# KleistLab/ADAPTed

Measured on AMD Instinct MI355X. Metric: reads/sec (adapter+polyA detect), RNA004 200k-sample reads, higher is better.
Workload: dtype f32 samples/statistics, f64 cumulative sums + LLR trace

## Files before the change

### adapted_amd/csrc/adapted_hip.hip

```cpp
#include <hip/hip_runtime.h>

#include <cmath>
#include <cstdio>
#include <cstring>
#include <cstdlib>
#include <string>
#include <vector>

#include "adapted_hip.h"
#include "handle.h"
#include "common.h"
__device__ unsigned long long g_dbg[ADP_NDBG] = {0};
__device__ unsigned long long g_bs_tally[ADP_NTALLY][8] = {{0}};
#include "llr_stream.h"
#include "n1_select.h"
#include "n1_fused.h"
#include "peaks.h"
#include "synth.h"
#include "validate.h"
#include "cand_stats2.h"
#include "series_pipe.h"
#include "cnn_topk.h"
#include "cnn_conv.h"
#include "cnn_conv_split.h"
// ... 64 lines not shown
    bad |= h->sp.ensure(R * sizeof(SpOut));
    bad |= h->any_none.ensure(64);
    h->vstride = ((h->m + 63) / 64) * 64;
    {
        size_t cap = (size_t)10000000000ull / ((size_t)8 * h->vstride);
        if (cap < 256) cap = 256;
        size_t want = R < 1024 * VAL_WPE ? R : 1024 * VAL_WPE;
        h->vslots = (int)(want < cap ? want : cap);
    }
    bad |= h->vscratch.ensure((size_t)h->vslots * 2 * h->vstride * 4);
    h->pslots = (int)(R < 8192 ? R : 8192);
    if (llr) {
    bad |= h->pk.ensure(R * (Lp / 2 + 1) * 4);
    if (env_int("ADP_PK_VALUES", 1)) bad |= h->pkv.ensure(R * (Lp / 2 + 1) * 8);
    bad |= h->npk.ensure(R * 4);
    bad |= h->mk.ensure((size_t)h->pslots * (Lp / 2 + 1) * 4);
    }
    ALLOCCHK(bad);
    return 0;
}

template <class SRC>
__global__ void __launch_bounds__(256) k_expand_ragged(const SRC *__restrict__ packed, const int64_t *__restrict__ offs,
                                                        const int32_t *__restrict__ full_len, const float *__restrict__ scale,
                                                        const float *__restrict__ offset, int m, float *__restrict__ out)
{
    const int r = blockIdx.y;
    const int i0 = (blockIdx.x * 256 + threadIdx.x) * 4;
    if (i0 >= m) return;
    const int len = full_len[r] < m ? (full_len[r] > 0 ? full_len[r] : 0) : m;
// ... 421 lines not shown
static inline SigIdx sig_subset(const SigF32 &s, const int32_t *sel) { return SigIdx{s.base, sel}; }
static inline SigIdxI16 sig_subset(const SigI16 &s, const int32_t *sel) { return SigIdxI16{s.base, s.scale, s.offset, s.full_len, sel}; }

static void launch_cumsum(adp_handle *h, int n)
{
    const int split = env_int("ADP_CUMSUM_GATHER", 1) != 0;
    hipLaunchKernelGGL(k_cumsum, dim3((n + 63) / 64), dim3(64), 0, h->stream, h->down.as<float>(), h->nvalid.as<int32_t>(), h->Lp, n,
                       h->nck, h->ck.as<double2>(), h->tail.as<double2>(), split);
    if (split)
        hipLaunchKernelGGL(k_cumsum_gather, dim3((n + 63) / 64), dim3(64), 0, h->stream, h->down.as<float>(), h->nvalid.as<int32_t>(), h->Lp, n,
                           h->nck, h->ck.as<double2>(), h->tail.as<double2>());
}

static int gains_tile_fast() { return env_int("ADP_GAINS_TILE_FAST", 1) != 0; }

static void launch_polya_peak(adp_handle *h, int n, int mbsize, const double *pkv)
{
    const int grid = n < h->pslots ? n : h->pslots;
    hipLaunchKernelGGL(k_polya_peak, dim3(grid), dim3(64), (size_t)(((h->Lp / 2 + 1) + 8) / 16 + 2) * 4, h->stream, h->trace.as<double>(), h->nvalid.as<int32_t>(), h->Lp,
                       h->bmax.as<double>(), h->bmin.as<double>(), h->nsum, h->adapter_idx.as<int32_t>(), n, mbsize, h->mbs.as<MbState>(),
                       h->pk.as<int32_t>(), h->mk.as<uint32_t>(), h->polya_idx.as<int32_t>(), h->npk.as<int32_t>(), pkv, env_int("ADP_PK_PREFIX", PK_PREFIX));
}

template <class SIG>
static int llr_enqueue(adp_handle *h, SIG dsig, const int32_t *dlen, int n, int m, int minibatch, int flags,
                       adp_row *rows_dev, int rows_kind , int32_t *mb_status_dev, double *mb_params_dev,
                       int upto, const PhaseSync *ps)
{
    int rc = 0;
    const int n_mb = (n + minibatch - 1) / minibatch;
    h->last_n = n; h->last_nmb = n_mb;
    ALLOCCHK(h->mbs.ensure((size_t)n_mb * sizeof(MbState)) || h->ghist.ensure((size_t)n_mb * N1_BINS * 4) || h->gbelow.ensure((size_t)n_mb * 8) || h->gcnt.ensure((size_t)n_mb * 8 * N1_NCNT));
    rc = alloc_all(h, n, true);
    if (rc) return rc;
    hipStream_t st = h->stream;
#ifdef ADP_ABLATE
// ... 66 lines not shown
        }
        if (upto >= 4) {
            Scope s(h, "k_gains<1>");
            hipLaunchKernelGGL(k_gains<1>, dim3((n + GAINS_WPB - 1) / GAINS_WPB), dim3(64 * GAINS_WPB), 0, st, h->down.as<float>(), h->nvalid.as<int32_t>(), h->Lp, h->nck,
                               h->ck.as<double2>(), h->tail.as<double2>(), h->adapter_idx.as<int32_t>(), minibatch, mbs,
                               h->trace.as<double>(), h->bmax.as<double>(), h->bmin.as<double>(), h->nsum, h->t1.as<int2>(), 0, h->pk.as<int32_t>(), h->npk.as<int32_t>(), h->Lp / 2 + 1, h->gstat.as<double>(), n, h->oh1, nullptr, gains_tile_fast());
        }
        if (upto >= 5) {
            Scope s(h, "k_adapter_peak");
            hipLaunchKernelGGL(k_adapter_peak, dim3(n), dim3(64), 0, st, h->trace.as<double>(), h->nvalid.as<int32_t>(), h->Lp,
                               h->bmax.as<double>(), h->bmin.as<double>(), h->nsum, h->t1.as<int2>(), minibatch, mbs,
                               h->cfg.adapter_peak_prominence, h->cfg.adapter_peak_rel_height,
                               h->cfg.adapter_peak_width / h->ds, h->adapter_idx.as<int32_t>(), h->gstat.as<double>());
        }
        double *pkvp = (env_int("ADP_PK_VALUES", 1) && h->pkv.cap >= (size_t)n * (h->Lp / 2 + 1) * 8) ? h->pkv.as<double>() : nullptr;
        if (upto >= 6) {
            Scope s(h, "k_gains<2>");
            hipLaunchKernelGGL(k_gains<2>, dim3((n + GAINS_WPB - 1) / GAINS_WPB), dim3(64 * GAINS_WPB), 0, st, h->down.as<float>(), h->nvalid.as<int32_t>(), h->Lp, h->nck,
                               h->ck.as<double2>(), h->tail.as<double2>(), h->adapter_idx.as<int32_t>(), minibatch, mbs,
                               h->trace.as<double>(), h->bmax.as<double>(), h->bmin.as<double>(), h->nsum, h->t1.as<int2>(), 0, h->pk.as<int32_t>(), h->npk.as<int32_t>(), h->Lp / 2 + 1, h->gstat.as<double>(), n, 5, pkvp, gains_tile_fast());
        }
        if (upto >= 7) {
            Scope s(h, "k_polya_peak");
            launch_polya_peak(h, n, minibatch, pkvp);
        }
        if (ps && ps->done[1]) HIPCHK(hipEventRecord(ps->done[1], st));
    }
    if (upto >= 8) {
        if (ps && ps->wait[2]) HIPCHK(hipStreamWaitEvent(st, ps->wait[2], 0));
        if (h->L > 0)
            hipLaunchKernelGGL(k_llr_bounds, dim3((n + 255) / 256), dim3(256), 0, st, h->adapter_idx.as<int32_t>(),
                               h->polya_idx.as<int32_t>(), n, h->ds, h->pos_off, h->bounds.as<int64_t>(), h->topk_none.as<int8_t>(), h->layout == ADP_LAYOUT_SINGLE_READ ? 1 : 0);
        rc = launch_validate(h, dsig, dlen, n, m, 1, minibatch, true);
        if (rc) return rc;
        if (flags & ADP_WITH_START_PEAK) {
            if (sp_forked) HIPCHK(hipStreamWaitEvent(st, h->ev_join, 0));
            else if (!sp_done) {
                Scope s(h, "k_start_peak");
                hipLaunchKernelGGL(k_start_peak<SIG>, dim3(n), dim3(64), (size_t)64 * h->cfg.sp_downscale_factor * 4, st, dsig, dlen, n, m, h->cfg, h->sp.as<SpOut>());
// ... 1415 lines not shown
        if (bytes < 12) return ADP_ERR_INVALID;
        int32_t c[3] = {0, 0, 0};
        if (h->pt_looked) { HIPCHK(hipMemcpyAsync(c, phase_counts(h, OPW_PT), 12, hipMemcpyDeviceToHost, h->stream)); HIPCHK(hipStreamSynchronize(h->stream)); }
        memcpy(host_out, c, 12); return ADP_OK; }
    case 9: src = h->have_series.p; if (bytes > h->have_series.cap) return ADP_ERR_INVALID; break;
    case 13: src = h->ck.p; if (bytes > h->ck.cap) return ADP_ERR_INVALID; break;
    case 14: src = h->tail.p; if (bytes > h->tail.cap) return ADP_ERR_INVALID; break;
    case 15: src = h->bmax.p; if (bytes > h->bmax.cap) return ADP_ERR_INVALID; break;
    case 16: src = h->bmin.p; if (bytes > h->bmin.cap) return ADP_ERR_INVALID; break;
    case 17: src = h->gstat.p; if (bytes > h->gstat.cap) return ADP_ERR_INVALID; break;
    case 18: src = h->npk.p; if (bytes > h->npk.cap) return ADP_ERR_INVALID; break;
    case 19: src = h->pk.p; if (bytes > h->pk.cap) return ADP_ERR_INVALID; break;
    case 20:
        if (!h->pkv.p) { g_err = "this handle keeps no heights beside its maxima lists (ADP_PK_VALUES=0)"; return ADP_ERR_INVALID; }
        src = h->pkv.p; if (bytes > h->pkv.cap) return ADP_ERR_INVALID; break;
    case 21: {
        if (h->last_grouped || !h->mbs.p || h->last_nmb < 1 || bytes > (uint64_t)h->last_nmb * 4 || h->gbelow.cap < (size_t)h->last_nmb * 4) return ADP_ERR_INVALID;
        hipLaunchKernelGGL(k_mb_status_out, dim3((h->last_nmb + 255) / 256), dim3(256), 0, h->stream, h->mbs.as<MbState>(), h->last_nmb, h->gbelow.as<int32_t>());
        src = h->gbelow.p; break; }
    case 8: { if (bytes < 64 || bytes > sizeof(unsigned long long) * ADP_NDBG) return ADP_ERR_INVALID;
              HIPCHK(hipMemcpyFromSymbol(host_out, HIP_SYMBOL(g_dbg), bytes, 0, hipMemcpyDeviceToHost));
              static unsigned long long tally[ADP_NTALLY][8];
              HIPCHK(hipMemcpyFromSymbol(tally, HIP_SYMBOL(g_bs_tally), sizeof(tally), 0, hipMemcpyDeviceToHost));
              unsigned long long *o = (unsigned long long *)host_out;
              for (int j = 0; j < 5; j++) { o[j] = 0; for (int i = 0; i < ADP_NTALLY; i++) o[j] += tally[i][j]; }
              return ADP_OK; }
    default: return ADP_ERR_INVALID;
    }
    if (!src || (what != 0 && h->last_grouped)) { g_err = "no stage buffers of a plain (one-group) LLR call on this handle"; return ADP_ERR_INVALID; }
    HIPCHK(hipMemcpyAsync(host_out, src, bytes, hipMemcpyDeviceToHost, h->stream));
// ... 7 lines not shown
```

### adapted_amd/csrc/find_peaks.h

```cpp
#pragma once
#include "common.h"

#define DBLMAX 1.7976931348623157e308

template <class P>
struct TraceViewT {
    P x;
    P bmax;
    P bmin;
    int lo, hi;
    int sanitize;
};
typedef TraceViewT<const double *> TraceView;
typedef TraceViewT<const LDS double *> TraceViewL;

template <class TV>
static __device__ __forceinline__ double tv_get(const TV &t, int i)
{
    double v = t.x[i];
    if (t.sanitize) {
        if (v != v) v = 0.0;
        else if (__builtin_isinf(v)) v = v > 0 ? DBLMAX : -DBLMAX;
    }
    return v;
// ... 88 lines not shown
        if (m) {
            found = bstart + __ffsll((long long)m) - 1;
            if (KIND == WALK_PROM && in && e < found && v < lmn) lmn = v;
            break;
        }
        if (KIND == WALK_PROM && in && v < lmn) lmn = v;
        i = bstart + SUMBLK;
    }
    if (KIND == WALK_PROM) mn = wave_min(lmn);
    return found;
}

#ifndef WALK_CHUNK
#define WALK_CHUNK 4
#endif
enum { PB_DONE = 0, PB_LEFT = 1, PB_RIGHT = 2, PB_REJECT = 4 };
template <class TV>
static __device__ int tv_prominence_budget(const TV &t, int p, int budget, double pmin, double &prom, double &lmin_out, double &rmin_out)
{
    const double xp = tv_get(t, p);
    double left_min = xp, right_min = xp;
    int more = 0;
    bool stopped = false;
    for (int i0 = p, steps = 0; !stopped && i0 >= t.lo; i0 -= WALK_CHUNK, steps += WALK_CHUNK) {
        if (steps >= budget) { more |= PB_LEFT; break; }
        double v[WALK_CHUNK];
#pragma unroll
        for (int u = 0; u < WALK_CHUNK; u++) v[u] = (i0 - u >= t.lo) ? tv_get(t, i0 - u) : 0.0;
#pragma unroll
        for (int u = 0; u < WALK_CHUNK; u++) {
            if (!stopped) {
                if (i0 - u < t.lo || !(v[u] <= xp)) stopped = true;
                else if (v[u] < left_min) left_min = v[u];
            }
        }
    }
    if (!(more & PB_LEFT) && !(pmin <= xp - left_min)) return PB_REJECT;
    stopped = false;
    for (int i0 = p, steps = 0; !stopped && i0 <= t.hi; i0 += WALK_CHUNK, steps += WALK_CHUNK) {
        if (steps >= budget) { more |= PB_RIGHT; break; }
        double v[WALK_CHUNK];
#pragma unroll
        for (int u = 0; u < WALK_CHUNK; u++) v[u] = (i0 + u <= t.hi) ? tv_get(t, i0 + u) : 0.0;
#pragma unroll
        for (int u = 0; u < WALK_CHUNK; u++) {
            if (!stopped) {
                if (i0 + u > t.hi || !(v[u] <= xp)) stopped = true;
                else if (v[u] < right_min) right_min = v[u];
            }
        }
    }
    if (!(more & PB_RIGHT) && !(pmin <= xp - right_min)) return PB_REJECT;
    prom = xp - (left_min > right_min ? left_min : right_min);
    lmin_out = left_min; rmin_out = right_min;
    return more;
}
template <class TV>
static __device__ bool tv_width_budget(const TV &t, int p, double prom, double rel, int budget, double &width, double lmin, double rmin)
{
    const double xp = tv_get(t, p);
    const double height = xp - prom * rel;
    int il = t.lo;
    {
        bool stopped = false;
        for (int i0 = p, steps = 0; !stopped && i0 > t.lo; i0 -= WALK_CHUNK, steps += WALK_CHUNK) {
            if (steps >= budget) return false;
            double v[WALK_CHUNK];
#pragma unroll
            for (int u = 0; u < WALK_CHUNK; u++) v[u] = (i0 - u > t.lo) ? tv_get(t, i0 - u) : 0.0;
#pragma unroll
            for (int u = 0; u < WALK_CHUNK; u++) {
                if (!stopped) {
                    if (i0 - u <= t.lo) { stopped = true; il = t.lo; }
                    else if (!(height < v[u]) || v[u] == lmin) { stopped = true; il = i0 - u; }
                }
            }
        }
    }
    int ir = t.hi;
    {
        bool stopped = false;
        for (int i0 = p, steps = 0; !stopped && i0 < t.hi; i0 += WALK_CHUNK, steps += WALK_CHUNK) {
            if (steps >= budget) return false;
            double v[WALK_CHUNK];
#pragma unroll
            for (int u = 0; u < WALK_CHUNK; u++) v[u] = (i0 + u < t.hi) ? tv_get(t, i0 + u) : 0.0;
#pragma unroll
            for (int u = 0; u < WALK_CHUNK; u++) {
                if (!stopped) {
                    if (i0 + u >= t.hi) { stopped = true; ir = t.hi; }
                    else if (!(height < v[u]) || v[u] == rmin) { stopped = true; ir = i0 + u; }
                }
            }
        }
    }
    double left_ip = (double)il, right_ip = (double)ir;
    { double xi = tv_get(t, il); if (xi < height) left_ip += (height - xi) / (tv_get(t, il + 1) - xi); }
    { double xi = tv_get(t, ir); if (xi < height) right_ip -= (height - xi) / (tv_get(t, ir - 1) - xi); }
    width = right_ip - left_ip;
    return true;
}

#ifndef WALK_BUDGET
#define WALK_BUDGET 8
#endif
template <class TV>
static __device__ bool wave_peak_ok(const TV &t, int p, double pmin, double wmin, double rel)
{
    const int ln = lane_id();
    double prom = 0.0, lmn = 0.0, rmn = 0.0;
    bool have = p >= 0, done = true;
    int pb = PB_DONE;
    if (have) pb = tv_prominence_budget(t, p, WALK_BUDGET, pmin, prom, lmn, rmn);
    if (pb == PB_REJECT) have = false;
// ... 23 lines not shown
        const double xp = tv_get(t, pp);
        const double height = xp - pr * rel;
        double dummy;
        int il = coop_find_down<WALK_WIDTH>(t, pp, t.lo + 1, xp, height, dummy, sl);
        if (il < t.lo + 1) il = t.lo;
        int ir = coop_find_up<WALK_WIDTH>(t, pp, t.hi - 1, xp, height, dummy, sr);
        if (ir > t.hi - 1) ir = t.hi;
        double left_ip = (double)il, right_ip = (double)ir;
        { double xi = tv_get(t, il); if (xi < height) left_ip += (height - xi) / (tv_get(t, il + 1) - xi); }
        { double xi = tv_get(t, ir); if (xi < height) right_ip -= (height - xi) / (tv_get(t, ir - 1) - xi); }
        if (ln == src) width = right_ip - left_ip;
    }
    return cand && (wmin <= width);
}

template <class TV>
static __device__ int wave_first_peak(const TV &t, double pmin, double wmin, double rel)
{
    const int ln = lane_id();
    for (int base = t.lo + 1; base < t.hi; base += 64) {
        int i = base + ln;
        int p = (i < t.hi) ? tv_peak_at(t, i) : -1;
        const bool ok = wave_peak_ok(t, p, pmin, wmin, rel);
        unsigned long long mk = __ballot(ok);
        if (mk) return __shfl(p, __ffsll((long long)mk) - 1);
    }
    return -1;
}
```

### adapted_amd/csrc/handle.h

```cpp
#pragma once
#include <hip/hip_runtime.h>

#include <string>
#include <vector>

#include "adapted_hip.h"
#include "carve.h"

#define ADP_HIDDEN __attribute__((visibility("hidden")))

extern ADP_HIDDEN thread_local std::string g_err;

#define HIPCHK(expr)                                                                         \
    do {                                                                                     \
        hipError_t e_ = (expr);                                                              \
        if (e_ != hipSuccess) {                                                              \
            g_err = std::string(#expr) + ": " + hipGetErrorString(e_);                       \
            return ADP_ERR_HIP;                                                              \
        }                                                                                    \
    } while (0)
#define RCCHK(expr) do { int rc_ = (expr); if (rc_) return rc_; } while (0)
#define ALLOCCHK(failed) do { if (failed) { g_err = "device allocation failed"; return ADP_ERR_HIP; } } while (0)

struct DevBuf {
// ... 18 lines not shown
struct ProfEntry { const char *name; hipEvent_t a, b; };
#define ADP_MAX_LANES 4

struct adp_handle {
    int device = 0;
    hipStream_t stream = nullptr;
    hipStream_t stream3 = nullptr;
    hipEvent_t ev_copy[16] = {};
    hipStream_t stream2 = nullptr;
    hipEvent_t ev_fork = nullptr, ev_join = nullptr;
    hipEvent_t ev_conv[3] = {};
    adp_cfg cfg;
    int max_reads = 0, m = 0;
    int T = 0, off = 0, ds = 1, L = 0, Lp = 0, nck = 0, nsum = 0;
    DevBuf mbs, ghist, gbelow, gcnt, cbuf, fz, fcnt, n1heavy, ct_pk, ct_pv, ct_out, gstat, down, nvalid, ck, tail, trace, bmax, bmin, t1, adapter_idx, polya_idx;
    DevBuf bounds, topk_none, rows, preq, series, have_series, vscratch, pk, pkv, npk, mk, st, sp, any_none, sig_stage, len_stage, bounds_stage;
    int vslots = 0, vstride = 0, pslots = 0;
    bool profiling = false;
    std::vector<ProfEntry> prof;
    std::vector<hipEvent_t> ev_pool;
    size_t ev_used = 0;
    int last_n = 0, last_nmb = 0;
    int layout = 0;
    int oh1 = 5;
    int pos_off = 0;
    DevBuf rng0;
    DevBuf cnn_w, cnn_act[2], cnn_x, cnn_sc, ct_st, ct_lnz, ct_ap, cstat, op_arena, op_used, series_plan;
    DevBuf ws;
    DevBuf fb_sel, so_sel, pt_sel, sub_ws;
    unsigned int fb_n_sel = 0, so_n_sel = 0;
    bool pt_looked = false;
// ... 57 lines not shown
```

### adapted_amd/csrc/llr_stream.h

```cpp
#pragma once
#include <type_traits>
#include "common.h"
#include "log_cr.h"
#include "wave_stats.h"

extern __device__ unsigned long long g_dbg[ADP_NDBG];

#define NP_TILE 512
struct SpHead {
    int32_t valid, max_idx, a2, e0;
    float mx;
    int32_t op_end;
    int32_t op_head, op_body, hit;
    int32_t pad;
};

template <class SIG, bool SP = false, int NQ = 0>
__global__ void __launch_bounds__(256) k_norm_pool(SIG sig, int m, int T, int off, int ds, int L, int Lp,
                                                   int mbsize, const MbState *__restrict__ mbs,
                                                   float *__restrict__ down, int32_t *__restrict__ nvalid,
                                                   const int64_t *__restrict__ ranges, const int32_t *__restrict__ full_len,
                                                   int tails_nan = 0, SpHead *__restrict__ sp_head = nullptr, float sp_thr = 0.f)
{
    extern __shared__ __attribute__((aligned(16))) float tile[];
// ... 323 lines not shown
#endif
#ifndef GAINS_EU
#define GAINS_EU 4
#endif
#ifndef GAINS_WPB
#define GAINS_WPB 4
#endif
template <int PASS>
__global__ void __launch_bounds__(64 * GAINS_WPB, 4) k_gains(const float *__restrict__ down, const int32_t *__restrict__ nvalid, int Lp, int nck,
                                              const double2 *__restrict__ ck, const double2 *__restrict__ tail,
                                              const int32_t *__restrict__ adapter_idx, int mbsize,
                                              const MbState *__restrict__ mbs, double *__restrict__ trace,
                                              double *__restrict__ bmax, double *__restrict__ bmin, int nsum,
                                              int2 *__restrict__ t1, int sanitize, int32_t *__restrict__ pk_all,
                                              int32_t *__restrict__ npk_all, int pk_stride, double *__restrict__ gstat, int n_reads, int oh1,
                                              double *__restrict__ pkv_all = nullptr, int tile_fast = 0)
{
    __shared__ __attribute__((aligned(16))) double sg_[GAINS_WPB][64 * (CK + 1)];
    __shared__ __attribute__((aligned(16))) double lt_[3 * LOGCR_N];
    LDS double *sg = (LDS double *)sg_[threadIdx.x >> 6];
    const int r = blockIdx.x * GAINS_WPB + (threadIdx.x >> 6);
    const int ln = lane_id();
    for (int i = threadIdx.x; i < 3 * LOGCR_N; i += 64 * GAINS_WPB) lt_[i] = g_logcr_table[i];
    __syncthreads();
    if (r >= n_reads) return;
    const LDS double *lt = (const LDS double *)lt_;
    auto flog = [&](double v) { return log_cr_impl(v, lt, [](double u) { return gains_log_slow(u); }); };
    if (mbs[r / mbsize].status != ADP_MB_OK) return;
    const int n = nvalid[r];
    if (n <= 0) return;
    int start = 0, oh = oh1, ot = 5;
    if (PASS == 2) {
        start = adapter_idx[r];
        if (start < 0) return;
        oh = 1; ot = 1;
    }
    const int E = n - 1;
    const float *s = down + (size_t)r * Lp;
    const double2 *c = ck + (size_t)r * nck;
// ... 11 lines not shown
    {
        double v = (start == E) ? 0.0 : var_seg(te.y, c2s, te.x, cs, (double)(E - start));
        vs = (double)(E - start) * flog(v);
    }
    const bool fast_read = tile_fast && __all(__builtin_fabs(vs) < __builtin_inf() && __builtin_bit_cast(uint64_t, vs) != 0x8000000000000000ULL);
    int n_fast = 0, n_redo = 0;
    int first_pos = 0x7fffffff, last_pos = -1;
    double st_s1 = 0.0, st_s2 = 0.0;
    int st_nan = 0;
    const bool emit = (PASS == 2 || sanitize) && pk_all;
    int32_t *pk = emit ? pk_all + (size_t)r * pk_stride : nullptr;
    double *pkv = (emit && pkv_all) ? pkv_all + (size_t)r * pk_stride : nullptr;
    int npk = 0;
    bool plateau = false;
    double carry1 = 0.0, carry2 = 0.0;
    for (int tb = 0; tb < n; tb += TRACE_TILE) {
        ws_sync();
        const int i0 = tb + ln * CK;
        const float4 *s4 = reinterpret_cast<const float4 *>(s + (i0 < Lp ? i0 : 0));
        double a = 0.0, b = 0.0;
        if (i0 < n) { double2 p = c[i0 / CK]; a = p.x; b = p.y; }
        double mx = -__builtin_inf(), mn = __builtin_inf();
        double dlh = (double)(i0 - start), dlt = (double)(E - i0);
        auto point = [&](auto interior_c, int t, int i, float qf) {
            constexpr bool INTERIOR = decltype(interior_c)::value;
            double gi = 0.0;
            const double lh_len = dlh, lt_len = dlt;
            dlh += 1.0; dlt -= 1.0;
            if (INTERIOR || i < n) {
                if (INTERIOR || (i >= start + oh && i < E - ot)) {
                    double vh = var_seg(b, c2s, a, cs, lh_len);
// ... 210 lines not shown
```

### adapted_amd/csrc/peaks.h

```cpp
#pragma once
#include "common.h"
#include "find_peaks.h"

extern __device__ unsigned long long g_dbg[ADP_NDBG];

template <class P>
static __device__ int adapter_peak_read(P g, P bmx, P bmn, int n, int2 se, double s1, double s2, int nnan,
                                        double prominence, double rel_height, int width)
{
    const int ln = lane_id();
    const int cn = se.y - se.x;
    if (n < 3 || cn < 3) return -1;
    double o1 = 0.0, o2 = 0.0; int onan = 0;
    for (int i0 = 0; i0 < se.x; i0 += 512) {
        double v[8];
#pragma unroll
        for (int u = 0; u < 8; u++) { const int i = i0 + u * 64 + ln; v[u] = i < se.x ? g[i] : 0.0; }
#pragma unroll
        for (int u = 0; u < 8; u++) { o1 += v[u]; o2 += v[u] * v[u]; }
    }
    for (int i0 = se.y; i0 < n; i0 += 512) {
        double v[8];
#pragma unroll
        for (int u = 0; u < 8; u++) { const int i = i0 + u * 64 + ln; v[u] = i < n ? g[i] : 0.0; }
// ... 58 lines not shown
#define PK_STEP 16
#endif
#ifndef PK_PREFIX
#define PK_PREFIX 224
#endif
#define PST_NONE 0u
#define PST_REMOVED 1u
#define PST_KEPT 2u
#define PST_UNDECIDED 3u

__global__ void __launch_bounds__(64, 8) k_polya_peak(const double *__restrict__ trace, const int32_t *__restrict__ nvalid, int Lp,
                                                   const double *__restrict__ bmax, const double *__restrict__ bmin, int nsum,
                                                   const int32_t *__restrict__ adapter_idx, int n_reads, int mbsize,
                                                   const MbState *__restrict__ mbs, int32_t *__restrict__ pk_all,
                                                   uint32_t *__restrict__ mk_all, int32_t *__restrict__ polya_idx,
                                                   const int32_t *__restrict__ npk_all, const double *__restrict__ pkv_all, int prefix)
{
    extern __shared__ __attribute__((aligned(16))) uint32_t stw_raw[];
    LDS uint32_t *stw = (LDS uint32_t *)stw_raw;
    const int ln = lane_id();
    const int half = Lp / 2 + 1;
    uint32_t *mk = mk_all + (size_t)blockIdx.x * half;
    for (int r = blockIdx.x; r < n_reads; r += gridDim.x) {
        int32_t *pk = pk_all + (size_t)r * half;
        int result = 0;
        const int n = nvalid[r];
        const bool active = mbs[r / mbsize].status == ADP_MB_OK && adapter_idx[r] >= 0 && n >= 3;
        if (active) {
            const double *g = trace + (size_t)r * Lp;
            TraceView tv{g, bmax + (size_t)r * nsum, bmin + (size_t)r * nsum, 0, n - 1, 1};
            int npk = npk_all[r];
            const bool recount = npk < 0;
            const double *pkv = (pkv_all && !recount) ? pkv_all + (size_t)r * half : nullptr;
            if (recount) npk = 0;
            double carry = 0.0;
            __syncthreads();
            for (int base0 = 0; recount && base0 < n; base0 += 256) {
                double vv[4], ee[4];
#pragma unroll
                for (int u = 0; u < 4; u++) {
                    const int i = base0 + u * 64 + ln;
                    vv[u] = (i < n) ? tv_get(tv, i) : 0.0;
                    ee[u] = (ln == 63 && i + 1 < n) ? tv_get(tv, i + 1) : 0.0;
                }
#pragma unroll
                for (int u = 0; u < 4; u++) {
                    const int base = base0 + u * 64;
                    if (base >= n) break;
                    const int i = base + ln;
                    const double v = vv[u];
                    double prev = __shfl_up(v, 1);
                    if (ln == 0) prev = carry;
                    double next = __shfl_down(v, 1);
                    if (ln == 63) next = ee[u];
                    carry = __shfl(v, 63);
                    int p = -1;
                    if (i > 0 && i < n - 1 && prev < v) {
                        if (next < v) p = i;
                        else if (next == v) {
                            int j = i + 1;
                            while (j < n - 1 && tv_get(tv, j) == v) j++;
                            if (tv_get(tv, j) < v) p = (i + j - 1) / 2;
                        }
                    }
                    unsigned long long m = __ballot(p >= 0);
                    if (p >= 0) pk[npk + __popcll(m & ((1ull << ln) - 1ull))] = p;
                    npk += __popcll(m);
                }
            }
            if (ABLATED(256)) npk = 0;
            int p0 = -1, p1 = -1;
            for (int attempt = 0; attempt < 2; attempt++) {
            const int wn = (attempt == 0 && prefix > 0 && npk > prefix) ? prefix : npk;
            __syncthreads();
            for (int w = ln; w < (wn + 8 + 15) / 16 + 1; w += 64) stw[w] = 0;
            __syncthreads();
            if (ln < 4 && wn + ln < npk) {
                const uint32_t sl = (uint32_t)(wn + ln + 4);
                __hip_atomic_fetch_or(&stw[sl >> 4], PST_UNDECIDED << ((sl & 15u) * 2u), __ATOMIC_RELAXED, __HIP_MEMORY_SCOPE_WORKGROUP);
            }
            int nund = 0;
            for (int base4 = 0; base4 < wn; base4 += 56 * 4) {
                int pp[4];
                double vv[4];
// ... 28 lines not shown
                    const double v = vv[u];
                    uint32_t mask = 0, lower = 0;
#pragma unroll
                    for (int j = 1; j <= 4; j++) {
                        const int pf = __shfl_down(p, j); const double vf = __shfl_down(v, j);
                        const bool within = pf - p <= 9;
                        if (within && vf >= v) mask |= 1u << (j - 1);
                        if (within && !(vf >= v)) lower |= 1u << (j - 1);
                    }
#pragma unroll
                    for (int j = 1; j <= 4; j++) {
                        const uint32_t lb = (uint32_t)__shfl_up((int)lower, j);
                        if (lb >> (j - 1) & 1u) mask |= 1u << (4 + j - 1);
                    }
                    const bool out = valid && ln >= 4 && ln < 60 && k < wn;
                    if (out) {
                        const uint32_t sl = (uint32_t)(k + 4);
                        __hip_atomic_fetch_or(&stw[sl >> 4], (mask ? PST_UNDECIDED : PST_KEPT) << ((sl & 15u) * 2u), __ATOMIC_RELAXED,
                                              __HIP_MEMORY_SCOPE_WORKGROUP);
                    }
                    const bool und = out && mask;
                    const unsigned long long m = __ballot(und);
                    if (und) mk[nund + __popcll(m & ((1ull << ln) - 1ull))] = ((uint32_t)k << 8) | mask;
                    nund += __popcll(m);
                }
            }
            __syncthreads();
            if (ABLATED(512)) nund = 0;
            while (nund > 0) {
                int w = 0;
                for (int base4 = 0; base4 < nund; base4 += 256) {
                    uint32_t ee[4];
#pragma unroll
                    for (int u = 0; u < 4; u++) { const int idx = base4 + 64 * u + ln; ee[u] = (idx < nund) ? mk[idx] : 0u; }
#pragma unroll
                    for (int u = 0; u < 4; u++) {
// ... 45 lines not shown
                    uint32_t stt = PST_NONE;
                    if (k < wn) {
                        const uint32_t sl = (uint32_t)(k + 4);
                        stt = (stw[sl >> 4] >> ((sl & 15u) * 2u)) & 3u;
                    }
                    const unsigned long long mu = __ballot(stt == PST_UNDECIDED);
                    if (mu && first_und == wn) first_und = base4 + 64 * u + __ffsll((long long)mu) - 1;
                    const bool kp = stt == PST_KEPT && k < first_und;
                    const unsigned long long m = __ballot(kp);
                    if (kp) kl[nkept + __popcll(m & ((1ull << ln) - 1ull))] = pq[u];
                    nkept += __popcll(m);
                }
            }
            __syncthreads();
            p0 = -1; p1 = -1;
            for (int base = 0; base < nkept && p1 < 0 && !ABLATED(1024); base += PK_STEP) {
                int k = base + ln;
                int i = (ln < PK_STEP && k < nkept) ? kl[k] : -1;
                const bool ok = wave_peak_ok(tv, i, 1.0, 10.0, 0.5);
                unsigned long long m = __ballot(ok);
                while (m && p1 < 0) {
                    int f = __ffsll((long long)m) - 1;
                    m &= m - 1;
                    int pi = __shfl(i, f);
                    if (p0 < 0) p0 = pi; else p1 = pi;
                }
            }
            if (p1 >= 0 || first_und >= npk) break;
            }
            if (p0 >= 0 && p1 < 0) result = p0;
            else if (p0 >= 0) {
                double h0 = g[p0], h1 = g[p1];
                if (h1 > h0) result = p1;
                else if (h1 < h0 * 0.5) result = p0;
                else {
                    double mv = __builtin_inf(); int mi = 0x7fffffff; int nan_i = 0x7fffffff;
                    for (int i = p0 + ln; i < p1; i += 64) {
                        double v = g[i];
                        if (v != v) nan_i = min(nan_i, i);
                        else if (v < mv) { mv = v; mi = i; }
                    }
                    nan_i = wave_min(nan_i);
                    double gm = wave_min(mv);
                    int cand = (mv == gm) ? mi : 0x7fffffff;
                    cand = wave_min(cand);
// ... 6 lines not shown
                    double xm = sx / cnt, ym = sy / cnt;
                    double sxx = 0, sxy = 0, syy = 0;
                    for (int i = idx_min + ln; i < p1; i += 64) {
                        double dx = (double)i - xm, dy = g[i] - ym;
                        sxx += dx * dx; sxy += dx * dy; syy += dy * dy;
                    }
                    sxx = wave_sum(sxx); sxy = wave_sum(sxy); syy = wave_sum(syy);
                    double inv = 1.0 / (double)cnt;
                    double ssxm = sxx * inv, ssxym = sxy * inv, ssym = syy * inv;
                    double rr;
                    if (ssxm == 0.0 || ssym == 0.0) rr = 0.0;
                    else { rr = ssxym / sqrt(ssxm * ssym); if (rr > 1.0) rr = 1.0; else if (rr < -1.0) rr = -1.0; }
                    result = (rr * rr >= 0.99) ? p1 : 0;
                }
            }
            __syncthreads();
        }
        if (ln == 0) polya_idx[r] = result;
    }
}
```

### adapted_amd/lib.py

```python
from __future__ import annotations

import ctypes as C
import operator
import os
import sys
from typing import List, Optional, Sequence

import numpy as np

from . import build as _build
from .container_types import DetectResults

_LIB = None

NCOL = 39
MAX_CAND = 16
MAX_OPEN_PORES = 16

ADP_IN_DEVICE, ADP_OUT_DEVICE, ADP_WITH_START_PEAK, ADP_TOPK_NONE, ADP_BOUNDS_HOST, ADP_TAILS_NAN = 1, 2, 4, 8, 16, 32
ADP_CNN_FALLBACK = 1 << 17
ADP_CNN_SECOND_LLR = 1 << 18
ADP_FLAG_TRUNCATED = 1 << 19
ADP_POLYA_TRUNCATED = 1 << 20
ROW_FROM_SECOND_LLR = 1
# ... 1235 lines not shown
    def debug_llr_upto(self, signals, full_lens, n, minibatch, stage, tails_nan: bool = False):
        sig, lens, flags = self._in(signals, full_lens, n, False)
        flags |= _flag_word(tails_nan=tails_nan)
        self._check(self.lib.adp_debug_llr_upto(self._h, sig, lens, n, self.m, int(minibatch), flags, int(stage)))

    def debug_fetch(self, what: int, n: int):
        lp = np.zeros(1, dtype=np.int32)
        self._check(self.lib.adp_debug_fetch(self._h, 6, lp, 4))
        Lp = int(lp[0])
        if what == 6:
            return Lp
        shapes = {1: ((n,), np.int32), 2: ((n, Lp), np.float32), 3: ((n, Lp), np.float64), 4: ((n,), np.int32),
                  5: ((n,), np.int32), 7: ((n, 2), np.int32), 9: ((n,), np.int8),
                  13: ((n, Lp // 16, 2), np.float64), 14: ((n, 2), np.float64), 15: ((n, Lp // 64), np.float64),
                  16: ((n, Lp // 64), np.float64), 17: ((n, 3), np.float64), 18: ((n,), np.int32),
                  19: ((n, Lp // 2 + 1), np.int32), 20: ((n, Lp // 2 + 1), np.float64), 21: ((n,), np.int32)}
        if what == 0:
            raise ValueError("use debug_norm_params")
        shp, dt = shapes[what]
        a = np.zeros(shp, dtype=dt)
        self._check(self.lib.adp_debug_fetch(self._h, what, a, a.nbytes))
        return a

    def debug_cnn_fallback(self):
        a = np.zeros(3, dtype=np.int32)
        self._check(self.lib.adp_debug_fetch(self._h, 10, a, a.nbytes))
        return tuple(int(v) for v in a)

    def debug_cnn_second_opinion(self):
        a = np.zeros(4, dtype=np.int32)
        self._check(self.lib.adp_debug_fetch(self._h, 11, a, a.nbytes))
# ... 17 lines not shown
```

Before: 1.077 million.

## Window the second gains pass and redo only reads with undecided polyA peaks

The second LLR gains pass now computes the trace only up to a fixed window past the adapter end. The polyA peak search runs on that truncated trace with window-aware prominence and width checks that can return an 'unknown' result. Reads whose answer cannot be decided inside the window go onto a redo list, and for those reads the full gains pass and peak search run again. This targets the cost of computing long traces past the likely polyA region, but it adds two extra kernel launches, a memset, atomics, and edge-case logic that could change results if the window checks are wrong.

```diff
diff --git a/adapted_amd/csrc/adapted_hip.hip b/adapted_amd/csrc/adapted_hip.hip
--- a/adapted_amd/csrc/adapted_hip.hip
+++ b/adapted_amd/csrc/adapted_hip.hip
@@ -102,6 +102,8 @@
     bad |= h->pk.ensure(R * (Lp / 2 + 1) * 4);
     if (env_int("ADP_PK_VALUES", 1)) bad |= h->pkv.ensure(R * (Lp / 2 + 1) * 8);
     bad |= h->npk.ensure(R * 4);
+    bad |= h->wend.ensure(R * 4);
+    bad |= h->redo.ensure((R + 1) * 4);
     bad |= h->mk.ensure((size_t)h->pslots * (Lp / 2 + 1) * 4);
     }
     ALLOCCHK(bad);
@@ -553,12 +555,29 @@
 
 static int gains_tile_fast() { return env_int("ADP_GAINS_TILE_FAST", 1) != 0; }
 
-static void launch_polya_peak(adp_handle *h, int n, int mbsize, const double *pkv)
+#define G2_WINDOW_DEFAULT 1024
+static int g2_window(int upto)
+{
+    const char *e = getenv("ADP_G2_WINDOW");
+    if (!e || !*e) return upto >= 8 ? G2_WINDOW_DEFAULT : 0;
+    const int w = env_int("ADP_G2_WINDOW", G2_WINDOW_DEFAULT);
+    return w < 0 ? 0 : (w > (1 << 28) ? (1 << 28) : w);
+}
+static void launch_gains2(adp_handle *h, int n, int mbsize, double *pkv, int win, const int32_t *redo)
+{
+    hipLaunchKernelGGL(k_gains<2>, dim3((n + GAINS_WPB - 1) / GAINS_WPB), dim3(64 * GAINS_WPB), 0, h->stream, h->down.as<float>(), h->nvalid.as<int32_t>(), h->Lp, h->nck,
+                       h->ck.as<double2>(), h->tail.as<double2>(), h->adapter_idx.as<int32_t>(), mbsize, h->mbs.as<MbState>(),
+                       h->trace.as<double>(), h->bmax.as<double>(), h->bmin.as<double>(), h->nsum, h->t1.as<int2>(), 0, h->pk.as<int32_t>(), h->npk.as<int32_t>(), h->Lp / 2 + 1, h->gstat.as<double>(), n, 5, pkv, gains_tile_fast(),
+                       win, h->wend.as<int32_t>(), redo);
+}
+
+static void launch_polya_peak(adp_handle *h, int n, int mbsize, const double *pkv, bool windowed = false, bool redo_pass = false)
 {
     const int grid = n < h->pslots ? n : h->pslots;
     hipLaunchKernelGGL(k_polya_peak, dim3(grid), dim3(64), (size_t)(((h->Lp / 2 + 1) + 8) / 16 + 2) * 4, h->stream, h->trace.as<double>(), h->nvalid.as<int32_t>(), h->Lp,
                        h->bmax.as<double>(), h->bmin.as<double>(), h->nsum, h->adapter_idx.as<int32_t>(), n, mbsize, h->mbs.as<MbState>(),
-                       h->pk.as<int32_t>(), h->mk.as<uint32_t>(), h->polya_idx.as<int32_t>(), h->npk.as<int32_t>(), pkv, env_int("ADP_PK_PREFIX", PK_PREFIX));
+                       h->pk.as<int32_t>(), h->mk.as<uint32_t>(), h->polya_idx.as<int32_t>(), h->npk.as<int32_t>(), pkv, env_int("ADP_PK_PREFIX", PK_PREFIX),
+                       (windowed || redo_pass) ? h->wend.as<int32_t>() : (const int32_t *)nullptr, (windowed || redo_pass) ? h->redo.as<int32_t>() : (int32_t *)nullptr, redo_pass ? 1 : 0);
 }
 
 template <class SIG>
@@ -655,15 +674,22 @@
                                h->cfg.adapter_peak_width / h->ds, h->adapter_idx.as<int32_t>(), h->gstat.as<double>());
         }
         double *pkvp = (env_int("ADP_PK_VALUES", 1) && h->pkv.cap >= (size_t)n * (h->Lp / 2 + 1) * 8) ? h->pkv.as<double>() : nullptr;
+        int win = g2_window(upto);
+        if (win > 0 && (win + 1 + TRACE_TILE - 1) / TRACE_TILE * TRACE_TILE >= h->L) win = 0;
         if (upto >= 6) {
+            if (win > 0) HIPCHK(hipMemsetAsync(h->redo.p, 0, 4, st));
             Scope s(h, "k_gains<2>");
-            hipLaunchKernelGGL(k_gains<2>, dim3((n + GAINS_WPB - 1) / GAINS_WPB), dim3(64 * GAINS_WPB), 0, st, h->down.as<float>(), h->nvalid.as<int32_t>(), h->Lp, h->nck,
-                               h->ck.as<double2>(), h->tail.as<double2>(), h->adapter_idx.as<int32_t>(), minibatch, mbs,
-                               h->trace.as<double>(), h->bmax.as<double>(), h->bmin.as<double>(), h->nsum, h->t1.as<int2>(), 0, h->pk.as<int32_t>(), h->npk.as<int32_t>(), h->Lp / 2 + 1, h->gstat.as<double>(), n, 5, pkvp, gains_tile_fast());
+            launch_gains2(h, n, minibatch, pkvp, win, nullptr);
         }
         if (upto >= 7) {
-            Scope s(h, "k_polya_peak");
-            launch_polya_peak(h, n, minibatch, pkvp);
+            { Scope s(h, "k_polya_peak");
+              launch_polya_peak(h, n, minibatch, pkvp, win > 0); }
+            if (win > 0) {
+                { Scope s(h, "k_gains<2> redo");
+                  launch_gains2(h, n, minibatch, pkvp, 0, h->redo.as<int32_t>()); }
+                { Scope s(h, "k_polya_peak redo");
+                  launch_polya_peak(h, n, minibatch, pkvp, false, true); }
+            }
         }
         if (ps && ps->done[1]) HIPCHK(hipEventRecord(ps->done[1], st));
     }
@@ -2109,6 +2135,8 @@
     case 20:
         if (!h->pkv.p) { g_err = "this handle keeps no heights beside its maxima lists (ADP_PK_VALUES=0)"; return ADP_ERR_INVALID; }
         src = h->pkv.p; if (bytes > h->pkv.cap) return ADP_ERR_INVALID; break;
+    case 22: src = h->wend.p; if (bytes > h->wend.cap) return ADP_ERR_INVALID; break;
+    case 23: src = h->redo.p; if (bytes > h->redo.cap) return ADP_ERR_INVALID; break;
     case 21: {
         if (h->last_grouped || !h->mbs.p || h->last_nmb < 1 || bytes > (uint64_t)h->last_nmb * 4 || h->gbelow.cap < (size_t)h->last_nmb * 4) return ADP_ERR_INVALID;
         hipLaunchKernelGGL(k_mb_status_out, dim3((h->last_nmb + 255) / 256), dim3(256), 0, h->stream, h->mbs.as<MbState>(), h->last_nmb, h->gbelow.as<int32_t>());
diff --git a/adapted_amd/csrc/find_peaks.h b/adapted_amd/csrc/find_peaks.h
--- a/adapted_amd/csrc/find_peaks.h
+++ b/adapted_amd/csrc/find_peaks.h
@@ -126,8 +126,8 @@
 #ifndef WALK_CHUNK
 #define WALK_CHUNK 4
 #endif
-enum { PB_DONE = 0, PB_LEFT = 1, PB_RIGHT = 2, PB_REJECT = 4 };
-template <class TV>
+enum { PB_DONE = 0, PB_LEFT = 1, PB_RIGHT = 2, PB_REJECT = 4, PB_OPEN = 8 };
+template <bool WIN = false, class TV>
 static __device__ int tv_prominence_budget(const TV &t, int p, int budget, double pmin, double &prom, double &lmin_out, double &rmin_out)
 {
     const double xp = tv_get(t, p);
@@ -149,6 +149,7 @@
     }
     if (!(more & PB_LEFT) && !(pmin <= xp - left_min)) return PB_REJECT;
     stopped = false;
+    bool higher = false;
     for (int i0 = p, steps = 0; !stopped && i0 <= t.hi; i0 += WALK_CHUNK, steps += WALK_CHUNK) {
         if (steps >= budget) { more |= PB_RIGHT; break; }
         double v[WALK_CHUNK];
@@ -157,17 +158,18 @@
 #pragma unroll
         for (int u = 0; u < WALK_CHUNK; u++) {
             if (!stopped) {
-                if (i0 + u > t.hi || !(v[u] <= xp)) stopped = true;
+                if (i0 + u > t.hi || !(v[u] <= xp)) { stopped = true; if (WIN && i0 + u <= t.hi) higher = true; }
                 else if (v[u] < right_min) right_min = v[u];
             }
         }
     }
-    if (!(more & PB_RIGHT) && !(pmin <= xp - right_min)) return PB_REJECT;
+    if (WIN && !(more & PB_RIGHT) && !higher) more |= PB_OPEN;
+    if (!(more & (WIN ? PB_RIGHT | PB_OPEN : PB_RIGHT)) && !(pmin <= xp - right_min)) return PB_REJECT;
     prom = xp - (left_min > right_min ? left_min : right_min);
     lmin_out = left_min; rmin_out = right_min;
     return more;
 }
-template <class TV>
+template <bool WIN = false, class TV>
 static __device__ bool tv_width_budget(const TV &t, int p, double prom, double rel, int budget, double &width, double lmin, double rmin)
 {
     const double xp = tv_get(t, p);
@@ -190,6 +192,7 @@
         }
     }
     int ir = t.hi;
+    bool crossed = false;
     {
         bool stopped = false;
         for (int i0 = p, steps = 0; !stopped && i0 < t.hi; i0 += WALK_CHUNK, steps += WALK_CHUNK) {
@@ -201,7 +204,7 @@
             for (int u = 0; u < WALK_CHUNK; u++) {
                 if (!stopped) {
                     if (i0 + u >= t.hi) { stopped = true; ir = t.hi; }
-                    else if (!(height < v[u]) || v[u] == rmin) { stopped = true; ir = i0 + u; }
+                    else if (!(height < v[u]) || v[u] == rmin) { stopped = true; ir = i0 + u; crossed = true; }
                 }
             }
         }
@@ -210,6 +213,7 @@
     { double xi = tv_get(t, il); if (xi < height) left_ip += (height - xi) / (tv_get(t, il + 1) - xi); }
     { double xi = tv_get(t, ir); if (xi < height) right_ip -= (height - xi) / (tv_get(t, ir - 1) - xi); }
     width = right_ip - left_ip;
+    if (WIN && !crossed) width = __builtin_nan("");
     return true;
 }
 
@@ -263,6 +267,93 @@
     return cand && (wmin <= width);
 }
 
+enum { PK3_FAIL = 0, PK3_PASS = 1, PK3_UNKNOWN = 2 };
+
+template <class TV>
+static __device__ double coop_width(const TV &t, int pp, double xp, double height, double sl, double sr, bool &crossed)
+{
+    double dummy;
+    int il = coop_find_down<WALK_WIDTH>(t, pp, t.lo + 1, xp, height, dummy, sl);
+    if (il < t.lo + 1) il = t.lo;
+    int ir = coop_find_up<WALK_WIDTH>(t, pp, t.hi - 1, xp, height, dummy, sr);
+    crossed = ir <= t.hi - 1;
+    if (!crossed) ir = t.hi;
+    double left_ip = (double)il, right_ip = (double)ir;
+    { double xi = tv_get(t, il); if (xi < height) left_ip += (height - xi) / (tv_get(t, il + 1) - xi); }
+    { double xi = tv_get(t, ir); if (xi < height) right_ip -= (height - xi) / (tv_get(t, ir - 1) - xi); }
+    return right_ip - left_ip;
+}
+
+template <class TV>
+static __device__ int wave_peak_ok_win(const TV &t, int p, double pmin, double wmin, double rel)
+{
+    const int ln = lane_id();
+    double prom = 0.0, lmn = 0.0, rmn = 0.0;
+    bool have = p >= 0;
+    int pb = PB_DONE;
+    if (have) pb = tv_prominence_budget<true>(t, p, WALK_BUDGET, pmin, prom, lmn, rmn);
+    if (pb == PB_REJECT) { have = false; pb = PB_DONE; }
+    unsigned long long todo = __ballot(have && (pb & (PB_LEFT | PB_RIGHT)));
+    while (todo) {
+        const int src = __ffsll((long long)todo) - 1;
+        todo &= todo - 1;
+        const int pp = __shfl(p, src), sides = __shfl(pb, src);
+        const double xp = tv_get(t, pp);
+        double lmin = __shfl(lmn, src), rmin = __shfl(rmn, src);
+        bool rej = false;
+        int open = sides & PB_OPEN;
+        if (sides & PB_LEFT) { coop_find_down<WALK_PROM>(t, pp, t.lo, xp, 0.0, lmin); rej = !(pmin <= xp - lmin); }
+        if (!rej && (sides & PB_RIGHT)) { if (coop_find_up<WALK_PROM>(t, pp, t.hi, xp, 0.0, rmin) > t.hi) open = PB_OPEN; }
+        if (ln == src) { if (rej) have = false; else { lmn = lmin; rmn = rmin; pb = open; } }
+    }
+    const double xpl = have ? tv_get(t, p) : 0.0;
+    const bool bounds = have && (pb & PB_OPEN) && rmn > lmn;
+    prom = xpl - (lmn > rmn ? lmn : rmn);
+    const bool cand = have && !bounds && (pmin <= prom);
+    int res = PK3_FAIL;
+    double width = 0.0;
+    bool done = true;
+    if (cand) done = tv_width_budget<true>(t, p, prom, rel, WALK_BUDGET, width, lmn, rmn);
+    todo = __ballot(cand && !done);
+    while (todo) {
+        const int src = __ffsll((long long)todo) - 1;
+        todo &= todo - 1;
+        const int pp = __shfl(p, src);
+        const double pr = __shfl(prom, src);
+        const double sl = __shfl(lmn, src), sr = __shfl(rmn, src);
+        const double xp = tv_get(t, pp);
+        bool crossed;
+        const double w = coop_width(t, pp, xp, xp - pr * rel, sl, sr, crossed);
+        if (ln == src) width = crossed ? w : __builtin_nan("");
+    }
+    if (cand) {
+        const double height = xpl - prom * rel;
+        if (width != width || ((pb & PB_OPEN) && !(rmn < height))) res = PK3_UNKNOWN;
+        else res = (wmin <= width) ? PK3_PASS : PK3_FAIL;
+    }
+    todo = __ballot(bounds);
+    while (todo) {
+        const int src = __ffsll((long long)todo) - 1;
+        todo &= todo - 1;
+        const int pp = __shfl(p, src);
+        const double sl = __shfl(lmn, src), sr = __shfl(rmn, src);
+        const double xp = tv_get(t, pp);
+        int rs = PK3_UNKNOWN;
+        bool crossed;
+        const double plo = xp - sr, phi = xp - sl;
+        if (pmin <= plo) {
+            const double hlo = xp - plo * rel;
+            if (sr < hlo) { const double w = coop_width(t, pp, xp, hlo, sl, sr, crossed); if (crossed && wmin <= w) rs = PK3_PASS; }
+        }
+        if (rs == PK3_UNKNOWN) {
+            const double w = coop_width(t, pp, xp, xp - phi * rel, sl, -__builtin_inf(), crossed);
+            if (crossed && w < wmin) rs = PK3_FAIL;
+        }
+        if (ln == src) res = rs;
+    }
+    return res;
+}
+
 template <class TV>
 static __device__ int wave_first_peak(const TV &t, double pmin, double wmin, double rel)
 {
diff --git a/adapted_amd/csrc/handle.h b/adapted_amd/csrc/handle.h
--- a/adapted_amd/csrc/handle.h
+++ b/adapted_amd/csrc/handle.h
@@ -56,7 +56,7 @@
     int max_reads = 0, m = 0;
     int T = 0, off = 0, ds = 1, L = 0, Lp = 0, nck = 0, nsum = 0;
     DevBuf mbs, ghist, gbelow, gcnt, cbuf, fz, fcnt, n1heavy, ct_pk, ct_pv, ct_out, gstat, down, nvalid, ck, tail, trace, bmax, bmin, t1, adapter_idx, polya_idx;
-    DevBuf bounds, topk_none, rows, preq, series, have_series, vscratch, pk, pkv, npk, mk, st, sp, any_none, sig_stage, len_stage, bounds_stage;
+    DevBuf bounds, topk_none, rows, preq, series, have_series, vscratch, pk, pkv, npk, wend, redo, mk, st, sp, any_none, sig_stage, len_stage, bounds_stage;
     int vslots = 0, vstride = 0, pslots = 0;
     bool profiling = false;
     std::vector<ProfEntry> prof;
diff --git a/adapted_amd/csrc/llr_stream.h b/adapted_amd/csrc/llr_stream.h
--- a/adapted_amd/csrc/llr_stream.h
+++ b/adapted_amd/csrc/llr_stream.h
@@ -361,15 +361,18 @@
                                               double *__restrict__ bmax, double *__restrict__ bmin, int nsum,
                                               int2 *__restrict__ t1, int sanitize, int32_t *__restrict__ pk_all,
                                               int32_t *__restrict__ npk_all, int pk_stride, double *__restrict__ gstat, int n_reads, int oh1,
-                                              double *__restrict__ pkv_all = nullptr, int tile_fast = 0)
+                                              double *__restrict__ pkv_all = nullptr, int tile_fast = 0, int win = 0,
+                                              int32_t *__restrict__ wend_all = nullptr, const int32_t *__restrict__ redo = nullptr)
 {
     __shared__ __attribute__((aligned(16))) double sg_[GAINS_WPB][64 * (CK + 1)];
     __shared__ __attribute__((aligned(16))) double lt_[3 * LOGCR_N];
     LDS double *sg = (LDS double *)sg_[threadIdx.x >> 6];
-    const int r = blockIdx.x * GAINS_WPB + (threadIdx.x >> 6);
+    int r = blockIdx.x * GAINS_WPB + (threadIdx.x >> 6);
     const int ln = lane_id();
+    if (PASS == 2 && redo && (int)(blockIdx.x * GAINS_WPB) >= redo[0]) return;
     for (int i = threadIdx.x; i < 3 * LOGCR_N; i += 64 * GAINS_WPB) lt_[i] = g_logcr_table[i];
     __syncthreads();
+    if (PASS == 2 && redo) { if (r >= redo[0]) return; r = redo[1 + r]; }
     if (r >= n_reads) return;
     const LDS double *lt = (const LDS double *)lt_;
     auto flog = [&](double v) { return log_cr_impl(v, lt, [](double u) { return gains_log_slow(u); }); };
@@ -411,7 +414,13 @@
     int npk = 0;
     bool plateau = false;
     double carry1 = 0.0, carry2 = 0.0;
-    for (int tb = 0; tb < n; tb += TRACE_TILE) {
+    int wend = n;
+    if (PASS == 2 && win > 0) {
+        const int we = (start + 1 + win + TRACE_TILE - 1) / TRACE_TILE * TRACE_TILE;
+        wend = we < n ? we : n;
+    }
+    if (PASS == 2 && wend_all && ln == 0) wend_all[r] = wend;
+    for (int tb = 0; tb < wend; tb += TRACE_TILE) {
         ws_sync();
         const int i0 = tb + ln * CK;
         const float4 *s4 = reinterpret_cast<const float4 *>(s + (i0 < Lp ? i0 : 0));
diff --git a/adapted_amd/csrc/peaks.h b/adapted_amd/csrc/peaks.h
--- a/adapted_amd/csrc/peaks.h
+++ b/adapted_amd/csrc/peaks.h
@@ -96,39 +96,47 @@
                                                    const int32_t *__restrict__ adapter_idx, int n_reads, int mbsize,
                                                    const MbState *__restrict__ mbs, int32_t *__restrict__ pk_all,
                                                    uint32_t *__restrict__ mk_all, int32_t *__restrict__ polya_idx,
-                                                   const int32_t *__restrict__ npk_all, const double *__restrict__ pkv_all, int prefix)
+                                                   const int32_t *__restrict__ npk_all, const double *__restrict__ pkv_all, int prefix,
+                                                   const int32_t *__restrict__ wend_all = nullptr, int32_t *__restrict__ redo = nullptr,
+                                                   int redo_pass = 0)
 {
     extern __shared__ __attribute__((aligned(16))) uint32_t stw_raw[];
     LDS uint32_t *stw = (LDS uint32_t *)stw_raw;
     const int ln = lane_id();
     const int half = Lp / 2 + 1;
     uint32_t *mk = mk_all + (size_t)blockIdx.x * half;
-    for (int r = blockIdx.x; r < n_reads; r += gridDim.x) {
+    int n_decided = 0, n_listed = 0;
+    const int n_work = redo_pass ? redo[0] : n_reads;
+    for (int wi = blockIdx.x; wi < n_work; wi += gridDim.x) {
+        const int r = redo_pass ? redo[1 + wi] : wi;
         int32_t *pk = pk_all + (size_t)r * half;
         int result = 0;
         const int n = nvalid[r];
         const bool active = mbs[r / mbsize].status == ADP_MB_OK && adapter_idx[r] >= 0 && n >= 3;
+        bool undecided = false;
         if (active) {
             const double *g = trace + (size_t)r * Lp;
-            TraceView tv{g, bmax + (size_t)r * nsum, bmin + (size_t)r * nsum, 0, n - 1, 1};
+            const int wend = (wend_all && !redo_pass) ? min(wend_all[r], n) : n;
+            const bool win = wend < n;
+            TraceView tv{g, bmax + (size_t)r * nsum, bmin + (size_t)r * nsum, 0, wend - 1, 1};
             int npk = npk_all[r];
             const bool recount = npk < 0;
             const double *pkv = (pkv_all && !recount) ? pkv_all + (size_t)r * half : nullptr;
             if (recount) npk = 0;
             double carry = 0.0;
             __syncthreads();
-            for (int base0 = 0; recount && base0 < n; base0 += 256) {
+            for (int base0 = 0; recount && base0 < wend; base0 += 256) {
                 double vv[4], ee[4];
 #pragma unroll
                 for (int u = 0; u < 4; u++) {
                     const int i = base0 + u * 64 + ln;
-                    vv[u] = (i < n) ? tv_get(tv, i) : 0.0;
-                    ee[u] = (ln == 63 && i + 1 < n) ? tv_get(tv, i + 1) : 0.0;
+                    vv[u] = (i < wend) ? tv_get(tv, i) : 0.0;
+                    ee[u] = (ln == 63 && i + 1 < wend) ? tv_get(tv, i + 1) : 0.0;
                 }
 #pragma unroll
                 for (int u = 0; u < 4; u++) {
                     const int base = base0 + u * 64;
-                    if (base >= n) break;
+                    if (base >= wend) break;
                     const int i = base + ln;
                     const double v = vv[u];
                     double prev = __shfl_up(v, 1);
@@ -137,12 +145,13 @@
                     if (ln == 63) next = ee[u];
                     carry = __shfl(v, 63);
                     int p = -1;
-                    if (i > 0 && i < n - 1 && prev < v) {
+                    if (i > 0 && i < wend - 1 && prev < v) {
                         if (next < v) p = i;
                         else if (next == v) {
                             int j = i + 1;
-                            while (j < n - 1 && tv_get(tv, j) == v) j++;
+                            while (j < wend - 1 && tv_get(tv, j) == v) j++;
                             if (tv_get(tv, j) < v) p = (i + j - 1) / 2;
+                            else if (win && tv_get(tv, j) == v) undecided = true;
                         }
                     }
                     unsigned long long m = __ballot(p >= 0);
@@ -150,6 +159,7 @@
                     npk += __popcll(m);
                 }
             }
+            undecided = __any(undecided);
             if (ABLATED(256)) npk = 0;
             int p0 = -1, p1 = -1;
             for (int attempt = 0; attempt < 2; attempt++) {
@@ -208,12 +218,13 @@
                         if (lb >> (j - 1) & 1u) mask |= 1u << (4 + j - 1);
                     }
                     const bool out = valid && ln >= 4 && ln < 60 && k < wn;
+                    const bool late = win && p >= wend - 10;
                     if (out) {
                         const uint32_t sl = (uint32_t)(k + 4);
-                        __hip_atomic_fetch_or(&stw[sl >> 4], (mask ? PST_UNDECIDED : PST_KEPT) << ((sl & 15u) * 2u), __ATOMIC_RELAXED,
+                        __hip_atomic_fetch_or(&stw[sl >> 4], ((mask || late) ? PST_UNDECIDED : PST_KEPT) << ((sl & 15u) * 2u), __ATOMIC_RELAXED,
                                               __HIP_MEMORY_SCOPE_WORKGROUP);
                     }
-                    const bool und = out && mask;
+                    const bool und = out && mask && !late;
                     const unsigned long long m = __ballot(und);
                     if (und) mk[nund + __popcll(m & ((1ull << ln) - 1ull))] = ((uint32_t)k << 8) | mask;
                     nund += __popcll(m);
@@ -289,21 +300,29 @@
             }
             __syncthreads();
             p0 = -1; p1 = -1;
-            for (int base = 0; base < nkept && p1 < 0 && !ABLATED(1024); base += PK_STEP) {
+            for (int base = 0; base < nkept && p1 < 0 && !undecided && !ABLATED(1024); base += PK_STEP) {
                 int k = base + ln;
                 int i = (ln < PK_STEP && k < nkept) ? kl[k] : -1;
-                const bool ok = wave_peak_ok(tv, i, 1.0, 10.0, 0.5);
-                unsigned long long m = __ballot(ok);
+                int ok3;
+                if (win) ok3 = wave_peak_ok_win(tv, i, 1.0, 10.0, 0.5);
+                else ok3 = wave_peak_ok(tv, i, 1.0, 10.0, 0.5) ? PK3_PASS : PK3_FAIL;
+                unsigned long long m = __ballot(ok3 != PK3_FAIL);
+                const unsigned long long unk = __ballot(ok3 == PK3_UNKNOWN);
                 while (m && p1 < 0) {
                     int f = __ffsll((long long)m) - 1;
                     m &= m - 1;
+                    if (unk >> f & 1ull) { undecided = true; break; }
                     int pi = __shfl(i, f);
                     if (p0 < 0) p0 = pi; else p1 = pi;
                 }
             }
-            if (p1 >= 0 || first_und >= npk) break;
-            }
-            if (p0 >= 0 && p1 < 0) result = p0;
+            if (p1 >= 0 || first_und >= npk || undecided) break;
+            }
+            if (win && p1 < 0) undecided = true;
+            if (undecided) {
+                n_listed++;
+                if (ln == 0) redo[1 + atomicAdd(&redo[0], 1)] = r;
+            } else if (p0 >= 0 && p1 < 0) result = p0;
             else if (p0 >= 0) {
                 double h0 = g[p0], h1 = g[p1];
                 if (h1 > h0) result = p1;
@@ -340,8 +359,11 @@
                     result = (rr * rr >= 0.99) ? p1 : 0;
                 }
             }
+            if (win && !undecided) n_decided++;
             __syncthreads();
         }
-        if (ln == 0) polya_idx[r] = result;
-    }
+        if (ln == 0 && !undecided) polya_idx[r] = result;
+    }
+    if (ln == 0 && n_decided) atomicAdd(&g_dbg[78], (unsigned long long)n_decided);
+    if (ln == 0 && n_listed) atomicAdd(&g_dbg[79], (unsigned long long)n_listed);
 }
diff --git a/adapted_amd/lib.py b/adapted_amd/lib.py
--- a/adapted_amd/lib.py
+++ b/adapted_amd/lib.py
@@ -1273,7 +1273,8 @@
                   5: ((n,), np.int32), 7: ((n, 2), np.int32), 9: ((n,), np.int8),
                   13: ((n, Lp // 16, 2), np.float64), 14: ((n, 2), np.float64), 15: ((n, Lp // 64), np.float64),
                   16: ((n, Lp // 64), np.float64), 17: ((n, 3), np.float64), 18: ((n,), np.int32),
-                  19: ((n, Lp // 2 + 1), np.int32), 20: ((n, Lp // 2 + 1), np.float64), 21: ((n,), np.int32)}
+                  19: ((n, Lp // 2 + 1), np.int32), 20: ((n, Lp // 2 + 1), np.float64), 21: ((n,), np.int32),
+                  22: ((n,), np.int32), 23: ((n + 1,), np.int32)}
         if what == 0:
             raise ValueError("use debug_norm_params")
         shp, dt = shapes[what]
```

New measurement: 1.193 million, median of 6. 10.8% higher.
